# bwfbowen/muax

Hardware: AMD Instinct MI355X
Metric: batched act() env-steps/sec at num_simulations=50 (higher is better)
Workload: dtype f32; 1 GPU; cartpole: 4096 roots/GPU, obs 4, MLP embed 8, A=2, support 10, num_simulations=50, dirichlet 0.25/0.3, tiebreak=threefry, temperature 1; roots_per_gpu=4096, num_simulations=50, parallelism=roots sharded x1, no collective, backend=none (one rank), launcher=none

## Files before the change

muax_amd/_jit.py:

```python
from __future__ import annotations

import ctypes as C
import hashlib
import os
import subprocess

from . import _build

JIT_DIR = os.path.join(_build.LIB_DIR, "jit")
_SOURCES = ["mz_fused_jit.hip", "mz_fused_group.inc", "mz_fused_launch.h", "mz_fused.cuh", "mz_spec.cuh", "mz_host.h"]
_loaded = {}
_failed = set()
_TRAIN_SOURCES = ["mz_train_jit.hip", "mz_train_launch.h", "mz_train.cuh", "mz_spec.cuh", "mz_host.h"]
PLAN_VERSION = 2
last_build_log = None


def _ceil_log2(n: int) -> int:
    return 0 if n <= 1 else 1 + _ceil_log2((n + 1) // 2)


def lds_bytes(A: int, E: int, NMAX: int, WAVES: int, long_paths: bool = False, gumbel: bool = True) -> int:
    selw = ((2 * A + 3) // 4) * 4
    st0 = selw + (4 if (gumbel or not long_paths) else 3)
    path0 = st0 + (5 if gumbel else 4) * A + (E if (E <= 16 and not long_paths) else 0)
    entry = 8 if _ceil_log2(NMAX) + max(1, _ceil_log2(A)) <= 8 else 16
    pathw = (NMAX * entry + 31) // 32
    ns = (path0 + (0 if long_paths else pathw)) | 1
    tree = ((ns * NMAX + 3) // 4) * 4 + (((A + 3) // 4) * 4 if (long_paths and gumbel) else 0)
# ... 214 lines not shown
```

muax_amd/csrc/mz_act.hip:

```cpp
#include <hip/hip_runtime.h>

#include <cstdlib>
#include <cstring>

#define MZ_NO_STEP_KERNELS
#include "mz_handle.h"
#include "mz_fused_launch.h"
#include "mz_wide_launch.h"

using mzh::fail;

template <class Call>
static int dispatch_with_scratch(mzs_handle* h, mz::FusedParams& p, int* rc, Call call) {
  const size_t BN = (size_t)h->cfg.batch * (h->cfg.num_simulations + 1);
  *rc = call();
  for (int tries = 0; tries < 2 && (*rc == mz::kNeedEmbScratch || *rc >= mz::kNeedPathScratch); ++tries) {
    if (*rc == mz::kNeedEmbScratch) {
      MZS_HIP(h, hipMalloc(reinterpret_cast<void**>(&h->fused_emb), BN * h->cfg.embed_dim * sizeof(float)));
      p.emb_scratch = h->fused_emb;
    } else {
      const int words = *rc - mz::kNeedPathScratch;
      if (h->fused_path) MZS_HIP(h, hipFree(h->fused_path));
      h->fused_path = nullptr;
      h->fused_path_words = 0;
// ... 16 lines not shown
  if (!h->have_weights) return fail(h, MZS_E_INVALID, "mzs_act_mlp: call mzs_mlp_set_weights first");
  if (!a->obs || !a->action || !a->action_weights || !a->root_value)
    return fail(h, MZS_E_INVALID, "mzs_act_mlp: obs/action/action_weights/root_value must be set");
  const mzs_config& c = h->cfg;
  if (c.policy == 0 && !a->dirichlet_noise && a->dirichlet_fraction != 0.0f)
    return fail(h, MZS_E_INVALID, "mzs_act_mlp: dirichlet_fraction != 0 needs dirichlet_noise");
  if (c.num_simulations > mz::kMaxSims) {
    if (h->allow_generic) return mzh::act_mlp_generic(h, a, stream_);
    return fail(h, MZS_E_UNSUPPORTED, "mzs_act_mlp: no fused kernel instance for num_simulations > 256; use the generic route "
                                      "(mzs_mlp_allow_generic) or the step-wise path");
  }
  hipStream_t stream = static_cast<hipStream_t>(stream_);
  MZS_HIP(h, hipSetDevice(c.device));

  mz::FusedParams p;
  memset(&p, 0, sizeof p);
  p.obs = a->obs; p.dirichlet_noise = a->dirichlet_noise; p.invalid = a->invalid_actions; p.gumbel = a->gumbel;
  const mzs_mlp_weights& w = h->w;
  mzh::copy_weights(w, p);
  p.action = a->action; p.action_weights = a->action_weights; p.root_value = a->root_value;
  p.search_value = a->search_value; p.depth_sum = a->depth_sum;
  if (a->tree) {
    const mzs_tree_view& t = *a->tree;
    const void* const* tp = reinterpret_cast<const void* const*>(&t);
    for (int i = 0; i < 12; ++i)
      if (!tp[i]) return fail(h, MZS_E_INVALID, "mzs_act_mlp: tree view has a null array");
    p.t_node_visits = t.node_visits; p.t_raw_values = t.raw_values; p.t_node_values = t.node_values;
    p.t_parents = t.parents; p.t_action_from_parent = t.action_from_parent;
    p.t_children_index = t.children_index; p.t_children_prior_logits = t.children_prior_logits;
    p.t_children_values = t.children_values; p.t_children_visits = t.children_visits;
    p.t_children_rewards = t.children_rewards; p.t_children_discounts = t.children_discounts;
// ... 6 lines not shown
  p.dirichlet_fraction = a->dirichlet_fraction; p.discount = w.discount; p.temperature = a->temperature;
  p.global_batch = (uint64_t)c.global_batch; p.root_offset = (uint64_t)c.root_offset;
  p.prof = h->prof;
  p.emb_scratch = p.export_tree ? nullptr : h->fused_emb;
  if (c.policy == 1) {
    if (!h->fused_table) {
      const std::vector<int32_t> table = mzh::visit_table(c.max_num_considered_actions, c.num_simulations);
      MZS_HIP(h, hipMalloc(reinterpret_cast<void**>(&h->fused_table), table.size() * sizeof(int32_t)));
      MZS_HIP(h, hipMemcpy(h->fused_table, table.data(), table.size() * sizeof(int32_t), hipMemcpyHostToDevice));
    }
    p.visit_table = h->fused_table;
    p.max_considered = c.max_num_considered_actions;
    p.gumbel_scale = c.gumbel_scale;
    mzh::h_split(a->key, 2, 1, p.k_gumbel);
  }
  mzh::derive_keys(a->key, h->cfg.num_simulations, h->k_sample, h->sim_keys.data());
  p.k_sample[0] = h->k_sample[0]; p.k_sample[1] = h->k_sample[1];
  memcpy(p.sim_keys, h->sim_keys.data(), sizeof(uint32_t) * 2 * (size_t)c.num_simulations);

  const int A = c.num_actions, E = c.embed_dim, F = 2 * w.support_size + 1, N = c.num_simulations + 1;
  p.F = F;
  const int mode = c.policy == 1 ? (c.qtransform == 1 ? 3 : 2) : (c.tiebreak ? 1 : 0);
  std::vector<mz::FusedDispatch> groups = {mz::fused_dispatch_g0, mz::fused_dispatch_g1, mz::fused_dispatch_g2,
                                           mz::fused_dispatch_g3, mz::fused_dispatch_g4};
  mz::jit_dispatchers(mode, &groups);
  if (h->allow_generic && getenv("MZS_FORCE_GENERIC") != nullptr) return mzh::act_mlp_generic(h, a, stream_);
  for (int compact = (c.batch > 16 * h->cu_count) ? 1 : 0; compact >= 0; --compact) {
    p.path_scratch = h->fused_path;
    p.path_words = h->fused_path_words;
    for (size_t gi = 0; gi < groups.size(); ++gi) {
      std::string err;
      int rc = 0;
      auto call = [&] { return groups[gi](mode, c.device, p, stream, A, E, F, N, compact != 0, &err); };
      if (int e = dispatch_with_scratch(h, p, &rc, call)) return e;
      if (rc == mz::kNoFusedInstance) continue;
      if (rc != MZS_OK) return fail(h, rc, "mzs_act_mlp: %s", err.c_str());
      return MZS_OK;
    }
  }
  if (mode >= 2 ? h->allow_wide_gumbel : h->allow_wide) {
    std::string err;
    int rc = 0;
    auto call = [&] { return mz::wide_dispatch(mode, h->allow_wide_gumbel, c.device, p, stream, A, E, F, &err); };
    if (int e = dispatch_with_scratch(h, p, &rc, call)) return e;
    if (rc == MZS_OK) return MZS_OK;
    if (rc != mz::kNoFusedInstance) return fail(h, rc, "mzs_act_mlp: %s", err.c_str());
  }
  if (h->allow_generic) return mzh::act_mlp_generic(h, a, stream_);
// ... 75 lines not shown
```

muax_amd/csrc/mz_api.hip:

```cpp
#include <hip/hip_runtime.h>

#include <cstdio>
#include <cstring>
#include <mutex>

#define MZ_NO_STEP_KERNELS
#include "mz_handle.h"
#include "mz_fused_launch.h"

namespace {

thread_local std::string g_create_error;

std::mutex g_jit_mutex;
std::vector<mz::FusedDispatch> g_jit_dispatch;
std::vector<mz::FusedDispatch> g_jit_dispatch_muzero;
struct JitTrain { int A, E, F; mzh::JitTrainLaunch launch; };
std::vector<JitTrain> g_jit_train;

}

int mzh::fail(mzs_handle* h, int code, const char* fmt, const char* a) {
  char buf[512];
  snprintf(buf, sizeof buf, fmt, a);
// ... 75 lines not shown
  return MZS_OK;
}
int mzs_mlp_allow_wide_gumbel(mzs_handle* h, int32_t allow) {
  if (!h) return MZS_E_INVALID;
  h->allow_wide_gumbel = allow != 0;
  return MZS_OK;
}

int mzs_destroy(mzs_handle* h) {
  if (!h) return MZS_OK;
  hipSetDevice(h->cfg.device);
  h->step.release();
  if (h->fused_table) hipFree(h->fused_table);
  if (h->fused_emb) hipFree(h->fused_emb);
  if (h->fused_path) hipFree(h->fused_path);
  if (h->jump_slab) hipFree(h->jump_slab);
  if (h->host_in) hipHostFree(h->host_in);
  if (h->host_out) hipHostFree(h->host_out);
  if (h->dev_noise) hipFree(h->dev_noise);
  if (h->gen_scratch) hipFree(h->gen_scratch);
  delete h;
  return MZS_OK;
}

int mzs_mlp_set_weights(mzs_handle* h, const mzs_mlp_weights* w) {
  if (!h) return MZS_E_INVALID;
  if (!w || w->struct_size != (int32_t)sizeof(mzs_mlp_weights))
    return fail(h, MZS_E_INVALID, "mzs_mlp_set_weights: null or size mismatch (ABI)");
  const float* const* ptrs = &w->repr_w;
  for (int i = 0; i < 18; ++i)
    if (!ptrs[i]) return fail(h, MZS_E_INVALID, "mzs_mlp_set_weights: null weight pointer");
  if (w->obs_dim <= 0 || w->support_size <= 0) return fail(h, MZS_E_INVALID, "mzs_mlp_set_weights: obs_dim/support_size");
  h->w = *w;
  h->have_weights = true;
  return MZS_OK;
}

static int register_dispatch(std::vector<mz::FusedDispatch>& list, void* dispatch, int32_t jit_abi) {
  if (!dispatch) return fail(nullptr, MZS_E_INVALID, "mzs_register_fused_dispatch: null");
  if (jit_abi != mzs_fused_jit_abi()) return fail(nullptr, MZS_E_INVALID, "mzs_register_fused_dispatch: the side library was built from other sources (ABI)");
  std::lock_guard<std::mutex> lock(g_jit_mutex);
  for (auto f : list)
    if (reinterpret_cast<void*>(f) == dispatch) return MZS_OK;
  list.push_back(reinterpret_cast<mz::FusedDispatch>(dispatch));
  return MZS_OK;
}
int mzs_register_fused_dispatch(void* dispatch, int32_t jit_abi) { return register_dispatch(g_jit_dispatch, dispatch, jit_abi); }
int mzs_register_fused_dispatch_muzero(void* dispatch, int32_t jit_abi) {
  return register_dispatch(g_jit_dispatch_muzero, dispatch, jit_abi);
// ... 4 lines not shown
```

muax_amd/csrc/mz_fused.cuh:

```cuda
#pragma once
#include "mz_spec.cuh"

#pragma clang fp contract(off)

namespace mz {

#ifdef MZ_PROFILE
#define MZ_TICK(slot)                                  \
  do {                                                 \
    uint64_t now_ = __builtin_amdgcn_s_memtime();      \
    prof_acc[slot] += now_ - prof_t;                   \
    prof_t = now_;                                     \
  } while (0)
#define MZ_TICKW(slot)                                 \
  do {                                                 \
    asm volatile("s_waitcnt vmcnt(0) lgkmcnt(0)" ::: "memory"); \
    MZ_TICK(slot);                                     \
  } while (0)
#else
#define MZ_TICK(slot) do {} while (0)
#define MZ_TICKW(slot) do {} while (0)
#endif

constexpr int kMaxSims = 256;
constexpr int kHidden = 16;

struct FusedParams {
  const float* obs;
  const float* dirichlet_noise;
  const uint8_t* invalid;
  const float* gumbel;
  const float *repr_w, *repr_b;
  const float *pv_w1, *pv_b1, *pv_w2, *pv_b2;
  const float *pp_w1, *pp_b1, *pp_w2, *pp_b2;
  const float *dr_w1, *dr_b1, *dr_w2, *dr_b2;
  const float *dn_w1, *dn_b1, *dn_w2, *dn_b2;
  int32_t* action;
  float* action_weights;
  float* root_value;
  float* search_value;
  int32_t* depth_sum;
  int32_t* t_node_visits; float* t_raw_values; float* t_node_values;
  int32_t* t_parents; int32_t* t_action_from_parent;
  int32_t* t_children_index; float* t_children_prior_logits; float* t_children_values;
  int32_t* t_children_visits; float* t_children_rewards; float* t_children_discounts;
  float* t_embeddings;
  float* emb_scratch;
  int32_t* path_scratch;
  int32_t B, obs_dim, S, max_depth, support, F, pred_on_parent, export_tree;
  float pb_c_init, pb_c_base, dirichlet_fraction, discount, temperature;
  uint64_t global_batch, root_offset;
  uint32_t k_sample[2];
  const int32_t* visit_table;
  int32_t max_considered;
  float gumbel_scale;
  uint32_t k_gumbel[2];
  uint32_t sim_keys[kMaxSims][2];
  uint64_t* prof;
  int32_t path_words;
};

template <int A_, int E_, int FS_, int NMAX_, int MODE_, int WAVES_ = 4, int REC_ = 0>
struct FusedCfg {
  static_assert(REC_ >= 0 && REC_ <= 2, "record kind");
  static constexpr bool PH_ = REC_ != 0;
  static constexpr bool PH = PH_;
  static constexpr bool LONG = REC_ == 2;
  static constexpr int WAVES = WAVES_, THREADS = 64 * WAVES_;
  static constexpr int A = A_, E = E_, FS = FS_, NMAX = NMAX_, MODE = MODE_;
  static_assert(FS_ == 2 || FS_ == 4, "support logits are handled as one or two packed pairs of lane slots");
  static constexpr bool TB = MODE_ == 1;
  static constexpr bool GUMBEL = MODE_ >= 2;
  static constexpr int QT = MODE_ == 3 ? 1 : 0;
  static constexpr int H = kHidden;
  static constexpr int ES = (E + 15) / 16;
  static constexpr bool L1_DPP = E_ > 16 && E_ % 8 == 0;
  static constexpr bool L2_BLOCK = L1_DPP && FS_ == 2 && (E_ + 15) / 16 == 2 && A_ <= 16;
  static constexpr bool PK = PH_ && E_ > 16 && !LONG;
  static_assert(!PK || (A_ <= 4 && NMAX_ <= 128 && MODE_ < 2), "packed record: four byte-sized children, MuZero policy");
  static constexpr int SEL0 = 0, SELW = PK ? 1 + A : ((2 * A + 3) / 4) * 4;
  static constexpr int HDR0 = SELW, JUMP = HDR0 + 2;
  static constexpr bool RAW_OK = !(PH_ && MODE_ != 3);
  static constexpr int HDRW = RAW_OK ? 4 : 3;
  static constexpr int ST0 = HDR0 + HDRW, STW = MODE_ >= 2 ? 5 : 4, ST_LOGIT = 4;
  static constexpr bool EMB_LDS = E_ <= 16 && !LONG;
  static constexpr int EMB0 = PK ? ST0 + 3 * A + 1 : ST0 + STW * A;
  static constexpr int off_score(int a) { return PK ? SEL0 + 1 + a : SEL0 + 2 * a + 1; }
  static constexpr int off_prob(int a) { return PK ? ST0 + a : ST0 + STW * a; }
  static constexpr int off_val(int a) { return PK ? ST0 + A + a : ST0 + STW * a + 1; }
  static constexpr int off_rew(int a) { return PK ? ST0 + 2 * A + a : ST0 + STW * a + 3; }
  static constexpr int off_logit(int a) { return ST0 + STW * a + ST_LOGIT; }
  static constexpr int VIS0 = ST0 + 3 * A;
  static MZ_DEV void load_cidx(const int* ndi, int (&cidx)[A]) {
// ... 60 lines not shown

template <int NIN, int NOUT>
struct RowLinear {
  static constexpr int IS = (NIN + 15) / 16, OS = (NOUT + 15) / 16;
  float w[NIN][OS];
  float b[OS];
  MZ_DEV void load(const float* __restrict__ W, const float* __restrict__ Bv, int j) {
#pragma unroll
    for (int t = 0; t < OS; ++t) {
      int k = j + 16 * t;
      b[t] = k < NOUT ? Bv[k] : 0.0f;
#pragma unroll
      for (int i = 0; i < NIN; ++i) w[i][t] = k < NOUT ? W[i * NOUT + k] : 0.0f;
    }
  }
  MZ_DEV void apply(const float (&x)[IS], float (&y)[OS]) const {
#pragma unroll
    for (int t = 0; t < OS; ++t) y[t] = 0.0f;
    StaticFor<0, NIN>::run([&](auto ic) {
      constexpr int i = decltype(ic)::value;
      float xb = bcast<(i & 15)>(x[i >> 4]);
#pragma unroll
      for (int t = 0; t < OS; ++t) y[t] = __builtin_fmaf(xb, w[i][t], y[t]);
    });
#pragma unroll
    for (int t = 0; t < OS; ++t) y[t] = y[t] + b[t];
  }
};

template <int NIN, int OS>
struct RowLinearRT {
  float w[NIN][OS];
  float b[OS];
  MZ_DEV void load(const float* __restrict__ W, const float* __restrict__ Bv, int j, int nout) {
#pragma unroll
    for (int t = 0; t < OS; ++t) {
      int k = j + 16 * t;
      b[t] = k < nout ? Bv[k] : 0.0f;
#pragma unroll
      for (int i = 0; i < NIN; ++i) w[i][t] = k < nout ? W[i * nout + k] : 0.0f;
    }
  }
};

template <int E, int A>
struct RowLinearOneHot2 {
  f32x2 w[E];
  f32x2 wa[A];
  f32x2 b;
  MZ_DEV void load(const float* __restrict__ W0, const float* __restrict__ B0, const float* __restrict__ W1,
                   const float* __restrict__ B1, int j) {
    b = (f32x2){B0[j], B1[j]};
    StaticFor<0, E>::run([&](auto ic) {
      constexpr int i = decltype(ic)::value;
      w[i] = (f32x2){W0[i * kHidden + j], W1[i * kHidden + j]};
    });
    StaticFor<0, A>::run([&](auto ac) {
      constexpr int a = decltype(ac)::value;
      wa[a] = (f32x2){W0[(E + a) * kHidden + j], W1[(E + a) * kHidden + j]};
    });
  }
};

template <int E>
struct RowLinearPair {
  f32x2 w[E];
  f32x2 b;
  MZ_DEV void load(const float* __restrict__ W0, const float* __restrict__ B0, const float* __restrict__ W1,
                   const float* __restrict__ B1, int j) {
    b = (f32x2){B0[j], B1[j]};
    StaticFor<0, E>::run([&](auto ic) {
      constexpr int i = decltype(ic)::value;
      w[i] = (f32x2){W0[i * kHidden + j], W1[i * kHidden + j]};
    });
  }
};

template <int N>
MZ_DEV void row_softmax(const float (&x)[(N + 15) / 16], int j, float (&p)[(N + 15) / 16]) {
  constexpr int NSLOT = (N + 15) / 16;
  constexpr int STEPS = N >= 16 ? 4 : ceil_log2(N);
  float m = -INFINITY;
#pragma unroll
  for (int t = 0; t < NSLOT; ++t) m = (j + 16 * t < N) ? fmaxf(m, x[t]) : m;
  m = row_max<STEPS>(m);
  float e[NSLOT];
  float part = 0.0f;
#pragma unroll
// ... 59 lines not shown
      s[0] = q.x;
      s[1] = q.y;
      return;
    }
  }
#pragma unroll
  for (int t = 0; t < NSLOT; ++t) s[t] = (s[t] - mn) / scale;
}

struct RowBias2 {
  f32x2 b;
  MZ_DEV void load(const float* __restrict__, const float* __restrict__ B0, const float* __restrict__,
                   const float* __restrict__ B1, int j) {
    b = (f32x2){B0[j], B1[j]};
  }
};

template <bool COND, class T, class F> struct PickType { using type = T; };
template <class T, class F> struct PickType<false, T, F> { using type = F; };

template <class C>
struct Nets {
  typename PickType<C::PK, RowBias2, RowLinearPair<C::E>>::type p1;
  RowLinearRT<kHidden, C::FS> pv2;
  RowLinear<kHidden, C::A> pp2;
  typename PickType<C::PK, RowBias2, RowLinearOneHot2<C::E, C::A>>::type d1;
  RowLinearRT<kHidden, C::FS> dr2;
  RowLinear<kHidden, C::E> dn2;
  const float* wlds = nullptr;

// ... 3 lines not shown
      for (int idx = tid; idx < (E / 2) * 16; idx += C::THREADS) {
        const int i = 2 * (idx >> 4), jj = idx & 15;
        *reinterpret_cast<float4*>(wl + 4 * idx) = make_float4(p.pv_w1[i * kHidden + jj], p.pp_w1[i * kHidden + jj],
                                                               p.pv_w1[(i + 1) * kHidden + jj], p.pp_w1[(i + 1) * kHidden + jj]);
      }
      float* wd = wl + C::W1P_WORDS;
      for (int idx = tid; idx < ((RD + 1) / 2) * 16; idx += C::THREADS) {
        const int i = 2 * (idx >> 4), jj = idx & 15;
        const bool two = i + 1 < RD;
        *reinterpret_cast<float4*>(wd + 4 * idx) = make_float4(p.dr_w1[i * kHidden + jj], p.dn_w1[i * kHidden + jj],
                                                               two ? p.dr_w1[(i + 1) * kHidden + jj] : 0.0f,
                                                               two ? p.dn_w1[(i + 1) * kHidden + jj] : 0.0f);
      }
    }
  }
  template <int WHICH>
  MZ_DEV f32x2 first_layers_lds(const float (&x)[C::ES]) const {
    static_assert(C::E % 8 == 0, "eight inputs per statement");
    const float* base = wlds + (WHICH ? C::W1P_WORDS : 0);
    float h0 = 0.0f, h1 = 0.0f;
    StaticFor<0, C::E / 8>::run([&](auto ic) {
      constexpr int i = 8 * decltype(ic)::value;
      f32x2 w[8];
#pragma unroll
      for (int q = 0; q < 4; ++q) {
        const float4 v = *reinterpret_cast<const float4*>(base + (i / 2 + q) * 64);
        w[2 * q] = (f32x2){v.x, v.y};
        w[2 * q + 1] = (f32x2){v.z, v.w};
      }
      fmac_bcast_pair8<(i & 15), (i & 15) == 0>(h0, h1, x[i >> 4], w);
// ... 2 lines not shown
  }
  MZ_DEV f32x2 first_p(const float (&x)[C::ES]) const {
    if constexpr (C::PK) return first_layers_lds<0>(x);
    else return first_layers(x, p1.w);
  }
  MZ_DEV f32x2 first_d(const float (&x)[C::ES]) const {
    if constexpr (C::PK) return first_layers_lds<1>(x);
    else return first_layers(x, d1.w);
  }

  MZ_DEV void load(const FusedParams& p, int j) {
    p1.load(p.pv_w1, p.pv_b1, p.pp_w1, p.pp_b1, j);
    pv2.load(p.pv_w2, p.pv_b2, j, p.F); pp2.load(p.pp_w2, p.pp_b2, j);
    d1.load(p.dr_w1, p.dr_b1, p.dn_w1, p.dn_b1, j);
    dr2.load(p.dr_w2, p.dr_b2, j, p.F); dn2.load(p.dn_w2, p.dn_b2, j);
  }
  template <class W>
  MZ_DEV f32x2 first_layers(const float (&x)[C::ES], const W& w) const {
    if constexpr (C::L1_DPP) {
      static_assert(C::E % 8 == 0, "eight inputs per statement");
      float h0 = 0.0f, h1 = 0.0f;
      StaticFor<0, C::E / 8>::run([&](auto ic) {
        constexpr int i = 8 * decltype(ic)::value;
        fmac_bcast_pair8<(i & 15), (i & 15) == 0>(h0, h1, x[i >> 4], &w[i]);
      });
      return (f32x2){h0, h1};
    } else {
      f32x2 h = splat2(0.0f);
      StaticFor<0, C::E>::run([&](auto ic) {
        constexpr int i = decltype(ic)::value;
// ... 323 lines not shown
    x[a] = logit[a] + qv[a];
    mxl = fmaxf(mxl, logit[a]);
  }
  softmax_inlane<A>(x, pr);
#pragma unroll
  for (int a = 0; a < A; ++a) {
    float r = fmaxf((gum[a] + (logit[a] - mxl)) + qv[a], -1e9f);
    r = r + (vis[a] == considered_visit ? 0.0f : -INFINITY);
    r = ((inv_bits >> a) & 1u) ? -INFINITY : r;
    const float in = pr[a] - (float)vis[a] / (float)(1 + sum_visits);
    sc[a] = is_root ? r : in;
  }
}

template <class C>
__global__ __launch_bounds__(C::THREADS, (C::PH && !C::LONG) ? 2 : 1) void mz_act_fused_kernel(const FusedParams p) {
  constexpr int A = C::A, E = C::E, NS = C::NS;
  extern __shared__ __attribute__((aligned(16))) float lds[];
  if constexpr (!C::PK) asm volatile("; keep AGPRs allocatable" ::: "a0");
  const int tid = threadIdx.x;
  const int lane = tid & 63;
  const int j = lane & 15;
  const int root_in_wg = (tid >> 6) * 4 + (lane >> 4);
  const int r_raw = blockIdx.x * C::ROOTS_PER_WG + root_in_wg;
  const int r = r_raw < p.B ? r_raw : p.B - 1;

#ifdef MZ_PROFILE
  uint64_t prof_acc[16] = {0, 0, 0, 0, 0, 0, 0, 0, 0, 0, 0, 0, 0, 0, 0, 0};
  uint64_t prof_t = __builtin_amdgcn_s_memtime();
#endif
  Nets<C> nets;
  if constexpr (C::PK) {
    nets.load(p, j);
    nets.wlds = lds + C::TBL_WORDS + 4 * j;
  }
  float* tbl = lds;
  for (int i = tid; i < C::TBL_WORDS / 2; i += C::THREADS) {
    tbl[2 * i] = puct_scale(i, p.pb_c_init, p.pb_c_base);
    tbl[2 * i + 1] = i > 0 ? 1.0f / (float)i : 0.0f;
  }
  Nets<C>::fill_lds(p, lds + C::TBL_WORDS, tid);
  __syncthreads();

  float* tree = lds + C::TBL_WORDS + C::WLDS_WORDS + root_in_wg * C::ROOT_WORDS;
  int* itree = reinterpret_cast<int*>(tree);
  const uint64_t rg = p.root_offset + (uint64_t)r;
  const int S = p.S;
  const int max_depth = p.max_depth > 0 ? p.max_depth : S;
  const int N = S + 1;
  const int support = p.support;
  const bool ex = p.export_tree != 0;

  float* gemb = C::EMB_LDS ? nullptr : (ex ? p.t_embeddings : p.emb_scratch) + (size_t)r * N * E;

  int32_t* gpath = C::PH ? p.path_scratch + (size_t)r * N * C::PATHW : nullptr;

  if constexpr (!C::PK) nets.load(p, j);
  {
    int4* q4 = reinterpret_cast<int4*>(itree);
    const int nq = (N * NS + 3) / 4;
    for (int q = j; q < nq; q += 16) q4[q] = make_int4(0, 0, 0, 0);
    for (int n = j; n < N; n += 16) {
      if constexpr (C::PK) itree[n * NS + C::SEL0] = -1;
      else {
#pragma unroll
        for (int a = 0; a < A; ++a) itree[n * NS + C::SEL0 + 2 * a] = -1;
      }
    }
  }
  if (ex) {
    for (int n = j; n < N; n += 16) {
      size_t o = (size_t)r * N + n;
      p.t_raw_values[o] = 0.0f;
      p.t_parents[o] = -1;
      p.t_action_from_parent[o] = -1;
    }
    for (int i = j; i < N * A; i += 16) p.t_children_prior_logits[(size_t)r * N * A + i] = 0.0f;
    if constexpr (!C::EMB_LDS)
      for (int i = j; i < N * E; i += 16) gemb[i] = 0.0f;
  }

  float s[C::ES];
  {
    const float* ob = p.obs + (size_t)r * p.obs_dim;
#pragma unroll
    for (int t = 0; t < C::ES; ++t) {
      int k = j + 16 * t;
      float acc = 0.0f;
      {
        const int kc = k < E ? k : 0;
        int i = 0;
        for (; i + 4 <= p.obs_dim; i += 4) {
          float o4[4], w4[4];
#pragma unroll
          for (int q = 0; q < 4; ++q) {
            o4[q] = ob[i + q];
            w4[q] = p.repr_w[(i + q) * E + kc];
          }
#pragma unroll
          for (int q = 0; q < 4; ++q) acc = __builtin_fmaf(o4[q], w4[q], acc);
        }
        for (; i < p.obs_dim; ++i) acc = __builtin_fmaf(ob[i], p.repr_w[i * E + kc], acc);
        acc = acc + p.repr_b[kc];
      }
      s[t] = k < E ? acc : 0.0f;
    }
    row_min_max_normalize<E>(s, j);
  }
  float v0, pl0;
  nets.predict(s, j, support, p.F, v0, pl0);
  uint32_t inv_bits = 0;
  if (p.invalid != nullptr) {
#pragma unroll
    for (int a = 0; a < A; ++a) inv_bits |= p.invalid[(size_t)r * A + a] ? (1u << a) : 0u;
  }
  int ncons = 0;
  int root_jw;
  {
    float lg, pq[1];
    if constexpr (!C::GUMBEL) {
      float x[1] = {pl0}, pr[1];
      row_softmax<A>(x, j, pr);
      float nz = (p.dirichlet_noise != nullptr && j < A) ? p.dirichlet_noise[(size_t)r * A + j] : 0.0f;
      float keep = 1.0f - p.dirichlet_fraction;
      float noisy = keep * pr[0] + p.dirichlet_fraction * nz;
      lg = log_pos(fmaxf(noisy, kFltTiny));
      if (p.invalid != nullptr) {
        float mx = row_max<4>(j < A ? lg : -INFINITY);
        lg = ((inv_bits >> j) & 1u) ? kFltLowest : lg - mx;
      }
      float lx[1] = {lg};
      row_softmax<A>(lx, j, pq);
    } else {
      lg = pl0;
      if (inv_bits != 0) {
        float mx = row_max<4>(j < A ? lg : -INFINITY);
        lg = ((inv_bits >> j) & 1u) ? kFltLowest : lg - mx;
      }
// ... 546 lines not shown
```

muax_amd/csrc/mz_fused_group.inc:

```
#include <mutex>

#ifndef MZ_INSTANCES_FILE
#define MZ_INSTANCES_FILE "mz_instances.def"
#endif
#include "../../include/mzsearch.h"
#include "mz_fused_launch.h"
#include "mz_host.h"

namespace mz {
namespace {

template <class C>
int launch_fused(int device, const FusedParams& p, hipStream_t stream, std::string* err) {
  static mzh::LdsGrant granted;
  if (!granted.covers(device, (size_t)C::LDS_BYTES)) {
    const hipError_t attr_err = hipFuncSetAttribute(reinterpret_cast<const void*>(&mz_act_fused_kernel<C>),
                                                    hipFuncAttributeMaxDynamicSharedMemorySize, C::LDS_BYTES);
    if (attr_err != hipSuccess) {
      *err = std::string("hipFuncSetAttribute: ") + hipGetErrorString(attr_err);
      return MZS_E_RUNTIME;
    }
    granted.note(device, (size_t)C::LDS_BYTES);
  }
  const int grid = (p.B + C::ROOTS_PER_WG - 1) / C::ROOTS_PER_WG;
  hipLaunchKernelGGL(mz_act_fused_kernel<C>, dim3(grid), dim3(C::THREADS), C::LDS_BYTES, stream, p);
  const hipError_t e = hipGetLastError();
  if (e != hipSuccess) {
    *err = std::string("fused kernel launch: ") + hipGetErrorString(e);
    return MZS_E_RUNTIME;
  }
  return MZS_OK;
}

#ifndef MZ_FUSED_MUZERO_ONLY
#define MZ_FUSED_MUZERO_ONLY 0
#endif

template <int A, int E, int FS, int NMAX, int WAVES, int PH>
int dispatch_mode(int mode, int device, const FusedParams& p, hipStream_t stream, std::string* err) {
  using C0 = FusedCfg<A, E, FS, NMAX, 0, WAVES, PH>;
  constexpr bool kMuZeroOnly = (PH && !C0::LONG) || MZ_FUSED_MUZERO_ONLY;
  if (kMuZeroOnly && mode >= 2) return kNoFusedInstance;
  if constexpr (PH) {
    if (p.path_scratch == nullptr || p.path_words < C0::PATHW) return kNeedPathScratch + C0::PATHW;
  }
  if constexpr (!C0::EMB_LDS) {
    if (!p.export_tree && p.emb_scratch == nullptr) return kNeedEmbScratch;
  }
  if constexpr (kMuZeroOnly) {
    if (mode == 1) return launch_fused<FusedCfg<A, E, FS, NMAX, 1, WAVES, PH>>(device, p, stream, err);
    return launch_fused<FusedCfg<A, E, FS, NMAX, 0, WAVES, PH>>(device, p, stream, err);
  } else {
    switch (mode) {
      case 3: return launch_fused<FusedCfg<A, E, FS, NMAX, 3, WAVES, PH>>(device, p, stream, err);
      case 2: return launch_fused<FusedCfg<A, E, FS, NMAX, 2, WAVES, PH>>(device, p, stream, err);
      case 1: return launch_fused<FusedCfg<A, E, FS, NMAX, 1, WAVES, PH>>(device, p, stream, err);
      default: return launch_fused<FusedCfg<A, E, FS, NMAX, 0, WAVES, PH>>(device, p, stream, err);
    }
  }
}

template <int G>
int dispatch_group(int mode, int device, const FusedParams& p, hipStream_t stream, int A, int E, int F, int N,
                   bool compact, std::string* err) {
#define MZS_INST(G_, A_, E_, FS_, NMAX_, WAVES_, PH_)                                                   \
  if constexpr (G_ == G)                                                                                \
    if (A == A_ && E == E_ && F > 16 * (FS_ - 2) && F > 16 && F <= 16 * FS_ && N <= NMAX_ &&                      \
        ((int)(PH_) == 2 ? !compact : compact == ((int)(PH_) == 1)))                                              \
      return dispatch_mode<A_, E_, FS_, NMAX_, WAVES_, PH_>(mode, device, p, stream, err);
#include MZ_INSTANCES_FILE
#undef MZS_INST
  return kNoFusedInstance;
}

}

#define MZ_CAT_(a, b) a##b
#define MZ_CAT(a, b) MZ_CAT_(a, b)
int MZ_CAT(fused_dispatch_g, MZ_FUSED_GROUP)(int mode, int device, const FusedParams& p, hipStream_t stream, int A, int E,
                                             int F, int N, bool compact, std::string* err) {
  return dispatch_group<MZ_FUSED_GROUP>(mode, device, p, stream, A, E, F, N, compact, err);
}

}
```

muax_amd/csrc/mz_fused_launch.h:

```cpp
#pragma once
#include <string>
#include <vector>

#include "mz_fused.cuh"

namespace mz {
constexpr int kNoFusedInstance = 1;
constexpr int kNeedPathScratch = 1000;
constexpr int kNeedEmbScratch = 2;
using FusedDispatch = int (*)(int mode, int device, const FusedParams& p, hipStream_t stream, int A, int E, int F,
                              int N, bool compact, std::string* err);
int fused_dispatch_g0(int mode, int device, const FusedParams& p, hipStream_t stream, int A, int E, int F, int N, bool compact, std::string* err);
int fused_dispatch_g1(int mode, int device, const FusedParams& p, hipStream_t stream, int A, int E, int F, int N, bool compact, std::string* err);
int fused_dispatch_g2(int mode, int device, const FusedParams& p, hipStream_t stream, int A, int E, int F, int N, bool compact, std::string* err);
int fused_dispatch_g3(int mode, int device, const FusedParams& p, hipStream_t stream, int A, int E, int F, int N, bool compact, std::string* err);
int fused_dispatch_g4(int mode, int device, const FusedParams& p, hipStream_t stream, int A, int E, int F, int N, bool compact, std::string* err);
void jit_dispatchers(int mode, std::vector<FusedDispatch>* out);
}
```

muax_amd/csrc/mz_handle.h:

```cpp
#pragma once
#include <string>
#include <vector>

#include "mz_host.h"
#include "mz_keys.h"
#include "mz_step_jump.cuh"

struct mzs_handle {
  mzs_config cfg;
  std::string err;
  bool have_weights = false;
  mzs_mlp_weights w;
  mz::StepState step;
  uint32_t k_sample[2] = {0, 0};
  std::vector<uint32_t> sim_keys;
  uint64_t* prof = nullptr;
  int32_t* fused_table = nullptr;
  float* fused_emb = nullptr;
  int32_t* fused_path = nullptr;
  int fused_path_words = 0;
  int cu_count = 0;
  void* host_in = nullptr; void* host_out = nullptr; void* dev_noise = nullptr;
  size_t host_in_bytes = 0;
  mz::JumpArgs jump = {nullptr, nullptr, nullptr, nullptr};
  void* jump_slab = nullptr;
  bool use_jump = false;
  int jump_roots = 0;
  bool allow_generic = false;
  float* gen_scratch = nullptr;
  bool allow_wide = false;
  bool allow_wide_gumbel = false;
};

namespace mzh {

// ... 13 lines not shown
```

muax_amd/csrc/mz_host.h:

```cpp
#pragma once
#include <hip/hip_runtime.h>

#include <atomic>
#include <cstdio>
#include <string>

#include "../../include/mzsearch.h"

#define MZS_HIP(h, call)                                                                            \
  do {                                                                                              \
    hipError_t e_ = (call);                                                                         \
    if (e_ != hipSuccess) return mzh::fail(h, MZS_E_RUNTIME, #call ": %s", hipGetErrorString(e_));  \
  } while (0)

namespace mz {
struct StepArgs;
struct JumpArgs;
}
namespace mzh {
int step_view(mzs_handle* h, mz::StepArgs* sa, mz::JumpArgs* ja, int* policy, const char* who, int* device = nullptr);
int fail(mzs_handle* h, int code, const char* fmt, const char* a = "");
using JitTrainLaunch = int (*)(const void* train_params, void* stream, char* err, int errlen);
JitTrainLaunch jit_train_instance(int A, int E, int F);
struct LdsGrant {
  std::atomic<size_t> have[64];
  bool covers(int device, size_t lds) const {
    return device >= 0 && device < 64 && have[device].load(std::memory_order_acquire) >= lds;
  }
  void note(int device, size_t lds) {
    if (device < 0 || device >= 64) return;
    size_t cur = have[device].load(std::memory_order_relaxed);
    while (cur < lds && !have[device].compare_exchange_weak(cur, lds, std::memory_order_release)) {
    }
  }
};
inline int check_device(int device, const char* who) {
  int ndev = 0;
  if (hipGetDeviceCount(&ndev) != hipSuccess || ndev <= 0)
    return fail(nullptr, MZS_E_NODEVICE, "%s: no HIP device (this library has no CPU fallback)", who);
  if (device < 0 || device >= ndev) return fail(nullptr, MZS_E_INVALID, "%s: bad device ordinal", who);
  return MZS_OK;
}
inline int select_device(int device, const char* who) {
  if (int rc = check_device(device, who)) return rc;
  MZS_HIP(nullptr, hipSetDevice(device));
  return MZS_OK;
}
}
```

Measured before the change: 34.77 million env-steps/s.

## Cache a prepacked weight and PUCT-table image across act calls

```diff
diff --git a/muax_amd/_jit.py b/muax_amd/_jit.py
--- a/muax_amd/_jit.py
+++ b/muax_amd/_jit.py
@@ -12,7 +12,7 @@
 _loaded = {}
 _failed = set()
 _TRAIN_SOURCES = ["mz_train_jit.hip", "mz_train_launch.h", "mz_train.cuh", "mz_spec.cuh", "mz_host.h"]
-PLAN_VERSION = 2
+PLAN_VERSION = 3
 last_build_log = None
 
 
diff --git a/muax_amd/csrc/mz_act.hip b/muax_amd/csrc/mz_act.hip
--- a/muax_amd/csrc/mz_act.hip
+++ b/muax_amd/csrc/mz_act.hip
@@ -1,5 +1,6 @@
 #include <hip/hip_runtime.h>
 
+#include <cstddef>
 #include <cstdlib>
 #include <cstring>
 
@@ -54,7 +55,7 @@
   MZS_HIP(h, hipSetDevice(c.device));
 
   mz::FusedParams p;
-  memset(&p, 0, sizeof p);
+  memset(&p, 0, offsetof(mz::FusedParams, sim_keys));
   p.obs = a->obs; p.dirichlet_noise = a->dirichlet_noise; p.invalid = a->invalid_actions; p.gumbel = a->gumbel;
   const mzs_mlp_weights& w = h->w;
   mzh::copy_weights(w, p);
@@ -91,9 +92,7 @@
     p.gumbel_scale = c.gumbel_scale;
     mzh::h_split(a->key, 2, 1, p.k_gumbel);
   }
-  mzh::derive_keys(a->key, h->cfg.num_simulations, h->k_sample, h->sim_keys.data());
-  p.k_sample[0] = h->k_sample[0]; p.k_sample[1] = h->k_sample[1];
-  memcpy(p.sim_keys, h->sim_keys.data(), sizeof(uint32_t) * 2 * (size_t)c.num_simulations);
+  mzh::derive_keys(a->key, c.num_simulations, p.k_sample, &p.sim_keys[0][0]);
 
   const int A = c.num_actions, E = c.embed_dim, F = 2 * w.support_size + 1, N = c.num_simulations + 1;
   p.F = F;
@@ -108,7 +107,7 @@
     for (size_t gi = 0; gi < groups.size(); ++gi) {
       std::string err;
       int rc = 0;
-      auto call = [&] { return groups[gi](mode, c.device, p, stream, A, E, F, N, compact != 0, &err); };
+      auto call = [&] { return groups[gi](mode, c.device, p, &h->fused_image, stream, A, E, F, N, compact != 0, &err); };
       if (int e = dispatch_with_scratch(h, p, &rc, call)) return e;
       if (rc == mz::kNoFusedInstance) continue;
       if (rc != MZS_OK) return fail(h, rc, "mzs_act_mlp: %s", err.c_str());
diff --git a/muax_amd/csrc/mz_api.hip b/muax_amd/csrc/mz_api.hip
--- a/muax_amd/csrc/mz_api.hip
+++ b/muax_amd/csrc/mz_api.hip
@@ -113,6 +113,7 @@
   if (h->fused_table) hipFree(h->fused_table);
   if (h->fused_emb) hipFree(h->fused_emb);
   if (h->fused_path) hipFree(h->fused_path);
+  if (h->fused_image.dev) hipFree(h->fused_image.dev);
   if (h->jump_slab) hipFree(h->jump_slab);
   if (h->host_in) hipHostFree(h->host_in);
   if (h->host_out) hipHostFree(h->host_out);
@@ -132,6 +133,7 @@
   if (w->obs_dim <= 0 || w->support_size <= 0) return fail(h, MZS_E_INVALID, "mzs_mlp_set_weights: obs_dim/support_size");
   h->w = *w;
   h->have_weights = true;
+  h->fused_image.valid = false;
   return MZS_OK;
 }
 
diff --git a/muax_amd/csrc/mz_fused.cuh b/muax_amd/csrc/mz_fused.cuh
--- a/muax_amd/csrc/mz_fused.cuh
+++ b/muax_amd/csrc/mz_fused.cuh
@@ -22,42 +22,53 @@
 #define MZ_TICKW(slot) do {} while (0)
 #endif
 
+#ifndef MZ_WEIGHTS_FIRST_PLAIN
+#define MZ_WEIGHTS_FIRST_PLAIN 0
+#endif
+#ifndef MZ_INPUTS_FIRST_PLAIN
+#define MZ_INPUTS_FIRST_PLAIN 0
+#endif
+#ifndef MZ_INPUTS_FIRST_PACKED
+#define MZ_INPUTS_FIRST_PACKED 0
+#endif
+
 constexpr int kMaxSims = 256;
 constexpr int kHidden = 16;
 
 struct FusedParams {
+  const float* image;
   const float* obs;
   const float* dirichlet_noise;
   const uint8_t* invalid;
   const float* gumbel;
+  int32_t* action;
+  float* action_weights;
+  float* root_value;
+  float* search_value;
+  int32_t* depth_sum;
+  int32_t B, obs_dim, S, max_depth, support, F, pred_on_parent, export_tree;
+  float pb_c_init, pb_c_base, dirichlet_fraction, discount, temperature;
+  int32_t path_words;
+  uint64_t global_batch, root_offset;
+  uint32_t k_sample[2];
+  float* emb_scratch;
+  int32_t* path_scratch;
+  const int32_t* visit_table;
+  int32_t max_considered;
+  float gumbel_scale;
+  uint32_t k_gumbel[2];
+  uint64_t* prof;
+  int32_t* t_node_visits; float* t_raw_values; float* t_node_values;
+  int32_t* t_parents; int32_t* t_action_from_parent;
+  int32_t* t_children_index; float* t_children_prior_logits; float* t_children_values;
+  int32_t* t_children_visits; float* t_children_rewards; float* t_children_discounts;
+  float* t_embeddings;
   const float *repr_w, *repr_b;
   const float *pv_w1, *pv_b1, *pv_w2, *pv_b2;
   const float *pp_w1, *pp_b1, *pp_w2, *pp_b2;
   const float *dr_w1, *dr_b1, *dr_w2, *dr_b2;
   const float *dn_w1, *dn_b1, *dn_w2, *dn_b2;
-  int32_t* action;
-  float* action_weights;
-  float* root_value;
-  float* search_value;
-  int32_t* depth_sum;
-  int32_t* t_node_visits; float* t_raw_values; float* t_node_values;
-  int32_t* t_parents; int32_t* t_action_from_parent;
-  int32_t* t_children_index; float* t_children_prior_logits; float* t_children_values;
-  int32_t* t_children_visits; float* t_children_rewards; float* t_children_discounts;
-  float* t_embeddings;
-  float* emb_scratch;
-  int32_t* path_scratch;
-  int32_t B, obs_dim, S, max_depth, support, F, pred_on_parent, export_tree;
-  float pb_c_init, pb_c_base, dirichlet_fraction, discount, temperature;
-  uint64_t global_batch, root_offset;
-  uint32_t k_sample[2];
-  const int32_t* visit_table;
-  int32_t max_considered;
-  float gumbel_scale;
-  uint32_t k_gumbel[2];
   uint32_t sim_keys[kMaxSims][2];
-  uint64_t* prof;
-  int32_t path_words;
 };
 
 template <int A_, int E_, int FS_, int NMAX_, int MODE_, int WAVES_ = 4, int REC_ = 0>
@@ -77,6 +88,8 @@
   static constexpr bool L1_DPP = E_ > 16 && E_ % 8 == 0;
   static constexpr bool L2_BLOCK = L1_DPP && FS_ == 2 && (E_ + 15) / 16 == 2 && A_ <= 16;
   static constexpr bool PK = PH_ && E_ > 16 && !LONG;
+  static constexpr bool WEIGHTS_FIRST = MZ_WEIGHTS_FIRST_PLAIN ? true : PK;
+  static constexpr bool INPUTS_FIRST = PK ? MZ_INPUTS_FIRST_PACKED : MZ_INPUTS_FIRST_PLAIN;
   static_assert(!PK || (A_ <= 4 && NMAX_ <= 128 && MODE_ < 2), "packed record: four byte-sized children, MuZero policy");
   static constexpr int SEL0 = 0, SELW = PK ? 1 + A : ((2 * A + 3) / 4) * 4;
   static constexpr int HDR0 = SELW, JUMP = HDR0 + 2;
@@ -167,6 +180,17 @@
       for (int i = 0; i < NIN; ++i) w[i][t] = k < NOUT ? W[i * NOUT + k] : 0.0f;
     }
   }
+  static constexpr int WORDS = (NIN + 1) * OS;
+  template <class V>
+  MZ_DEV void each(V& v) {
+#pragma unroll
+    for (int t = 0; t < OS; ++t) b[t] = v(b[t]);
+#pragma unroll
+    for (int i = 0; i < NIN; ++i) {
+#pragma unroll
+      for (int t = 0; t < OS; ++t) w[i][t] = v(w[i][t]);
+    }
+  }
   MZ_DEV void apply(const float (&x)[IS], float (&y)[OS]) const {
 #pragma unroll
     for (int t = 0; t < OS; ++t) y[t] = 0.0f;
@@ -192,6 +216,17 @@
       b[t] = k < nout ? Bv[k] : 0.0f;
 #pragma unroll
       for (int i = 0; i < NIN; ++i) w[i][t] = k < nout ? W[i * nout + k] : 0.0f;
+    }
+  }
+  static constexpr int WORDS = (NIN + 1) * OS;
+  template <class V>
+  MZ_DEV void each(V& v) {
+#pragma unroll
+    for (int t = 0; t < OS; ++t) b[t] = v(b[t]);
+#pragma unroll
+    for (int i = 0; i < NIN; ++i) {
+#pragma unroll
+      for (int t = 0; t < OS; ++t) w[i][t] = v(w[i][t]);
     }
   }
 };
@@ -213,6 +248,22 @@
       wa[a] = (f32x2){W0[(E + a) * kHidden + j], W1[(E + a) * kHidden + j]};
     });
   }
+  static constexpr int WORDS = 2 * (E + A + 1);
+  template <class V>
+  MZ_DEV void each(V& v) {
+    b.x = v(b.x);
+    b.y = v(b.y);
+    StaticFor<0, E>::run([&](auto ic) {
+      constexpr int i = decltype(ic)::value;
+      w[i].x = v(w[i].x);
+      w[i].y = v(w[i].y);
+    });
+    StaticFor<0, A>::run([&](auto ac) {
+      constexpr int a = decltype(ac)::value;
+      wa[a].x = v(wa[a].x);
+      wa[a].y = v(wa[a].y);
+    });
+  }
 };
 
 template <int E>
@@ -225,6 +276,17 @@
     StaticFor<0, E>::run([&](auto ic) {
       constexpr int i = decltype(ic)::value;
       w[i] = (f32x2){W0[i * kHidden + j], W1[i * kHidden + j]};
+    });
+  }
+  static constexpr int WORDS = 2 * (E + 1);
+  template <class V>
+  MZ_DEV void each(V& v) {
+    b.x = v(b.x);
+    b.y = v(b.y);
+    StaticFor<0, E>::run([&](auto ic) {
+      constexpr int i = decltype(ic)::value;
+      w[i].x = v(w[i].x);
+      w[i].y = v(w[i].y);
     });
   }
 };
@@ -314,6 +376,33 @@
                    const float* __restrict__ B1, int j) {
     b = (f32x2){B0[j], B1[j]};
   }
+  static constexpr int WORDS = 2;
+  template <class V>
+  MZ_DEV void each(V& v) {
+    b.x = v(b.x);
+    b.y = v(b.y);
+  }
+};
+
+struct ImagePut {
+  float* base;
+  int k = 0;
+  MZ_DEV float operator()(float x) {
+    base[(k >> 2) * 64 + (k & 3)] = x;
+    ++k;
+    return x;
+  }
+};
+struct ImageTake {
+  const float* base;
+  float4 cur = make_float4(0.0f, 0.0f, 0.0f, 0.0f);
+  int k = 0;
+  MZ_DEV float operator()(float) {
+    if ((k & 3) == 0) cur = *reinterpret_cast<const float4*>(base + (k >> 2) * 64);
+    const float x = (k & 3) == 0 ? cur.x : (k & 3) == 1 ? cur.y : (k & 3) == 2 ? cur.z : cur.w;
+    ++k;
+    return x;
+  }
 };
 
 template <bool COND, class T, class F> struct PickType { using type = T; };
@@ -347,6 +436,12 @@
       }
     }
   }
+  static MZ_DEV void copy_lds(const float* __restrict__ src, float* wl, int tid) {
+    if constexpr (C::PK) {
+      for (int idx = tid; idx < C::WLDS_WORDS / 4; idx += C::THREADS)
+        reinterpret_cast<float4*>(wl)[idx] = reinterpret_cast<const float4*>(src)[idx];
+    }
+  }
   template <int WHICH>
   MZ_DEV f32x2 first_layers_lds(const float (&x)[C::ES]) const {
     static_assert(C::E % 8 == 0, "eight inputs per statement");
@@ -379,6 +474,19 @@
     pv2.load(p.pv_w2, p.pv_b2, j, p.F); pp2.load(p.pp_w2, p.pp_b2, j);
     d1.load(p.dr_w1, p.dr_b1, p.dn_w1, p.dn_b1, j);
     dr2.load(p.dr_w2, p.dr_b2, j, p.F); dn2.load(p.dn_w2, p.dn_b2, j);
+  }
+  using P1 = typename PickType<C::PK, RowBias2, RowLinearPair<C::E>>::type;
+  using D1 = typename PickType<C::PK, RowBias2, RowLinearOneHot2<C::E, C::A>>::type;
+  static constexpr int WORDS = P1::WORDS + 2 * RowLinearRT<kHidden, C::FS>::WORDS + RowLinear<kHidden, C::A>::WORDS +
+                               D1::WORDS + RowLinear<kHidden, C::E>::WORDS;
+  static constexpr int CHUNKS = (WORDS + 3) / 4;
+  template <class V>
+  MZ_DEV void each(V& v) {
+    p1.each(v); pv2.each(v); pp2.each(v); d1.each(v); dr2.each(v); dn2.each(v);
+  }
+  MZ_DEV void load_image(const float* __restrict__ wimg, int j) {
+    ImageTake take{wimg + 4 * j};
+    each(take);
   }
   template <class W>
   MZ_DEV f32x2 first_layers(const float (&x)[C::ES], const W& w) const {
@@ -732,7 +840,49 @@
 }
 
 template <class C>
+struct FusedImage {
+  static constexpr int TBL0 = 0;
+  static constexpr int W0 = C::TBL_WORDS;
+  static constexpr int WL0 = W0 + Nets<C>::CHUNKS * 64;
+  static constexpr int REPR0 = WL0 + C::WLDS_WORDS;
+  static constexpr int REPR_ROWS = 16 * C::ES;
+  static_assert(W0 % 4 == 0 && WL0 % 4 == 0 && REPR0 % 4 == 0, "16-byte blocks");
+  static __host__ __device__ constexpr int repr_row_words(int obs_dim) { return 4 + ((obs_dim + 3) & ~3); }
+  static __host__ __device__ constexpr size_t words(int obs_dim) {
+    return (size_t)REPR0 + (size_t)REPR_ROWS * (size_t)repr_row_words(obs_dim);
+  }
+};
+
+template <class C>
+__global__ __launch_bounds__(C::THREADS) void mz_fused_image_kernel(const FusedParams p, float* __restrict__ img) {
+  using I = FusedImage<C>;
+  const int tid = threadIdx.x;
+  for (int i = tid; i < C::TBL_WORDS / 2; i += C::THREADS) {
+    img[I::TBL0 + 2 * i] = puct_scale(i, p.pb_c_init, p.pb_c_base);
+    img[I::TBL0 + 2 * i + 1] = i > 0 ? 1.0f / (float)i : 0.0f;
+  }
+  if (tid < 16) {
+    Nets<C> nets;
+    nets.load(p, tid);
+    ImagePut put{img + I::W0 + 4 * tid};
+    nets.each(put);
+  }
+  Nets<C>::fill_lds(p, img + I::WL0, tid);
+  const int rw = I::repr_row_words(p.obs_dim);
+  for (int idx = tid; idx < I::REPR_ROWS * rw; idx += C::THREADS) {
+    const int k = idx / rw, c = idx - k * rw;
+    float v = 0.0f;
+    if (k < C::E) {
+      if (c == 0) v = p.repr_b[k];
+      else if (c >= 4 && c - 4 < p.obs_dim) v = p.repr_w[(c - 4) * C::E + k];
+    }
+    img[I::REPR0 + idx] = v;
+  }
+}
+
+template <class C>
 __global__ __launch_bounds__(C::THREADS, (C::PH && !C::LONG) ? 2 : 1) void mz_act_fused_kernel(const FusedParams p) {
+  using I = FusedImage<C>;
   constexpr int A = C::A, E = C::E, NS = C::NS;
   extern __shared__ __attribute__((aligned(16))) float lds[];
   if constexpr (!C::PK) asm volatile("; keep AGPRs allocatable" ::: "a0");
@@ -747,17 +897,16 @@
   uint64_t prof_acc[16] = {0, 0, 0, 0, 0, 0, 0, 0, 0, 0, 0, 0, 0, 0, 0, 0};
   uint64_t prof_t = __builtin_amdgcn_s_memtime();
 #endif
+  const float* __restrict__ img = p.image;
   Nets<C> nets;
-  if constexpr (C::PK) {
-    nets.load(p, j);
-    nets.wlds = lds + C::TBL_WORDS + 4 * j;
+  if constexpr (C::WEIGHTS_FIRST) {
+    nets.load_image(img + I::W0, j);
+    if constexpr (C::PK) nets.wlds = lds + C::TBL_WORDS + 4 * j;
   }
   float* tbl = lds;
-  for (int i = tid; i < C::TBL_WORDS / 2; i += C::THREADS) {
-    tbl[2 * i] = puct_scale(i, p.pb_c_init, p.pb_c_base);
-    tbl[2 * i + 1] = i > 0 ? 1.0f / (float)i : 0.0f;
-  }
-  Nets<C>::fill_lds(p, lds + C::TBL_WORDS, tid);
+  for (int i = tid; i < C::TBL_WORDS / 4; i += C::THREADS)
+    reinterpret_cast<float4*>(tbl)[i] = reinterpret_cast<const float4*>(img + I::TBL0)[i];
+  Nets<C>::copy_lds(img + I::WL0, lds + C::TBL_WORDS, tid);
   __syncthreads();
 
   float* tree = lds + C::TBL_WORDS + C::WLDS_WORDS + root_in_wg * C::ROOT_WORDS;
@@ -773,7 +922,7 @@
 
   int32_t* gpath = C::PH ? p.path_scratch + (size_t)r * N * C::PATHW : nullptr;
 
-  if constexpr (!C::PK) nets.load(p, j);
+  if constexpr (!C::WEIGHTS_FIRST) nets.load_image(img + I::W0, j);
   {
     int4* q4 = reinterpret_cast<int4*>(itree);
     const int nq = (N * NS + 3) / 4;
@@ -798,6 +947,15 @@
       for (int i = j; i < N * E; i += 16) gemb[i] = 0.0f;
   }
 
+  uint32_t inv_bits = 0;
+  float nz = 0.0f;
+  if constexpr (C::INPUTS_FIRST) {
+    if (p.invalid != nullptr) {
+#pragma unroll
+      for (int a = 0; a < A; ++a) inv_bits |= p.invalid[(size_t)r * A + a] ? (1u << a) : 0u;
+    }
+    if constexpr (!C::GUMBEL) nz = (p.dirichlet_noise != nullptr && j < A) ? p.dirichlet_noise[(size_t)r * A + j] : 0.0f;
+  }
   float s[C::ES];
   {
     const float* ob = p.obs + (size_t)r * p.obs_dim;
@@ -806,20 +964,21 @@
       int k = j + 16 * t;
       float acc = 0.0f;
       {
-        const int kc = k < E ? k : 0;
+        const float* __restrict__ col = img + I::REPR0 + (size_t)k * I::repr_row_words(p.obs_dim);
+        const float bias = col[0];
         int i = 0;
         for (; i + 4 <= p.obs_dim; i += 4) {
-          float o4[4], w4[4];
-#pragma unroll
-          for (int q = 0; q < 4; ++q) {
-            o4[q] = ob[i + q];
-            w4[q] = p.repr_w[(i + q) * E + kc];
-          }
-#pragma unroll
-          for (int q = 0; q < 4; ++q) acc = __builtin_fmaf(o4[q], w4[q], acc);
+          float o4[4];
+#pragma unroll
+          for (int q = 0; q < 4; ++q) o4[q] = ob[i + q];
+          const float4 w4 = *reinterpret_cast<const float4*>(col + 4 + i);
+          acc = __builtin_fmaf(o4[0], w4.x, acc);
+          acc = __builtin_fmaf(o4[1], w4.y, acc);
+          acc = __builtin_fmaf(o4[2], w4.z, acc);
+          acc = __builtin_fmaf(o4[3], w4.w, acc);
         }
-        for (; i < p.obs_dim; ++i) acc = __builtin_fmaf(ob[i], p.repr_w[i * E + kc], acc);
-        acc = acc + p.repr_b[kc];
+        for (; i < p.obs_dim; ++i) acc = __builtin_fmaf(ob[i], col[4 + i], acc);
+        acc = acc + bias;
       }
       s[t] = k < E ? acc : 0.0f;
     }
@@ -827,10 +986,11 @@
   }
   float v0, pl0;
   nets.predict(s, j, support, p.F, v0, pl0);
-  uint32_t inv_bits = 0;
-  if (p.invalid != nullptr) {
-#pragma unroll
-    for (int a = 0; a < A; ++a) inv_bits |= p.invalid[(size_t)r * A + a] ? (1u << a) : 0u;
+  if constexpr (!C::INPUTS_FIRST) {
+    if (p.invalid != nullptr) {
+#pragma unroll
+      for (int a = 0; a < A; ++a) inv_bits |= p.invalid[(size_t)r * A + a] ? (1u << a) : 0u;
+    }
   }
   int ncons = 0;
   int root_jw;
@@ -839,7 +999,7 @@
     if constexpr (!C::GUMBEL) {
       float x[1] = {pl0}, pr[1];
       row_softmax<A>(x, j, pr);
-      float nz = (p.dirichlet_noise != nullptr && j < A) ? p.dirichlet_noise[(size_t)r * A + j] : 0.0f;
+      if constexpr (!C::INPUTS_FIRST) nz = (p.dirichlet_noise != nullptr && j < A) ? p.dirichlet_noise[(size_t)r * A + j] : 0.0f;
       float keep = 1.0f - p.dirichlet_fraction;
       float noisy = keep * pr[0] + p.dirichlet_fraction * nz;
       lg = log_pos(fmaxf(noisy, kFltTiny));
diff --git a/muax_amd/csrc/mz_fused_group.inc b/muax_amd/csrc/mz_fused_group.inc
--- a/muax_amd/csrc/mz_fused_group.inc
+++ b/muax_amd/csrc/mz_fused_group.inc
@@ -11,7 +11,43 @@
 namespace {
 
 template <class C>
-int launch_fused(int device, const FusedParams& p, hipStream_t stream, std::string* err) {
+int ensure_image(FusedParams& p, mzh::FusedImageSlot* slot, hipStream_t stream, std::string* err) {
+  static const char instance = 0;
+  if (!slot->serves(&instance, p.F, p.obs_dim, p.pb_c_init, p.pb_c_base)) {
+    const size_t words = FusedImage<C>::words(p.obs_dim);
+    slot->valid = false;
+    if (slot->cap_words < words) {
+      if (slot->dev) hipFree(slot->dev);
+      slot->dev = nullptr;
+      slot->cap_words = 0;
+      const hipError_t me = hipMalloc(reinterpret_cast<void**>(&slot->dev), words * sizeof(float));
+      if (me != hipSuccess) {
+        (void)hipGetLastError();
+        slot->dev = nullptr;
+        *err = std::string("launch image: hipMalloc: ") + hipGetErrorString(me);
+        return MZS_E_RUNTIME;
+      }
+      slot->cap_words = words;
+    }
+    hipError_t e = hipMemsetAsync(slot->dev, 0, words * sizeof(float), stream);
+    if (e == hipSuccess) {
+      float* img = slot->dev;
+      void* args[] = {&p, &img};
+      e = hipLaunchKernel(reinterpret_cast<const void*>(&mz_fused_image_kernel<C>), dim3(1), dim3(C::THREADS), args, 0, stream);
+    }
+    if (e != hipSuccess) {
+      (void)hipGetLastError();
+      *err = std::string("launch image build: ") + hipGetErrorString(e);
+      return MZS_E_RUNTIME;
+    }
+    slot->built(&instance, p.F, p.obs_dim, p.pb_c_init, p.pb_c_base);
+  }
+  p.image = slot->dev;
+  return MZS_OK;
+}
+
+template <class C>
+int launch_fused(int device, FusedParams& p, mzh::FusedImageSlot* slot, hipStream_t stream, std::string* err) {
   static mzh::LdsGrant granted;
   if (!granted.covers(device, (size_t)C::LDS_BYTES)) {
     const hipError_t attr_err = hipFuncSetAttribute(reinterpret_cast<const void*>(&mz_act_fused_kernel<C>),
@@ -22,10 +58,13 @@
     }
     granted.note(device, (size_t)C::LDS_BYTES);
   }
+  if (int rc = ensure_image<C>(p, slot, stream, err)) return rc;
   const int grid = (p.B + C::ROOTS_PER_WG - 1) / C::ROOTS_PER_WG;
-  hipLaunchKernelGGL(mz_act_fused_kernel<C>, dim3(grid), dim3(C::THREADS), C::LDS_BYTES, stream, p);
-  const hipError_t e = hipGetLastError();
+  void* args[] = {&p};
+  const hipError_t e = hipLaunchKernel(reinterpret_cast<const void*>(&mz_act_fused_kernel<C>), dim3(grid), dim3(C::THREADS),
+                                       args, C::LDS_BYTES, stream);
   if (e != hipSuccess) {
+    (void)hipGetLastError();
     *err = std::string("fused kernel launch: ") + hipGetErrorString(e);
     return MZS_E_RUNTIME;
   }
@@ -37,7 +76,7 @@
 #endif
 
 template <int A, int E, int FS, int NMAX, int WAVES, int PH>
-int dispatch_mode(int mode, int device, const FusedParams& p, hipStream_t stream, std::string* err) {
+int dispatch_mode(int mode, int device, FusedParams& p, mzh::FusedImageSlot* slot, hipStream_t stream, std::string* err) {
   using C0 = FusedCfg<A, E, FS, NMAX, 0, WAVES, PH>;
   constexpr bool kMuZeroOnly = (PH && !C0::LONG) || MZ_FUSED_MUZERO_ONLY;
   if (kMuZeroOnly && mode >= 2) return kNoFusedInstance;
@@ -48,26 +87,26 @@
     if (!p.export_tree && p.emb_scratch == nullptr) return kNeedEmbScratch;
   }
   if constexpr (kMuZeroOnly) {
-    if (mode == 1) return launch_fused<FusedCfg<A, E, FS, NMAX, 1, WAVES, PH>>(device, p, stream, err);
-    return launch_fused<FusedCfg<A, E, FS, NMAX, 0, WAVES, PH>>(device, p, stream, err);
+    if (mode == 1) return launch_fused<FusedCfg<A, E, FS, NMAX, 1, WAVES, PH>>(device, p, slot, stream, err);
+    return launch_fused<FusedCfg<A, E, FS, NMAX, 0, WAVES, PH>>(device, p, slot, stream, err);
   } else {
     switch (mode) {
-      case 3: return launch_fused<FusedCfg<A, E, FS, NMAX, 3, WAVES, PH>>(device, p, stream, err);
-      case 2: return launch_fused<FusedCfg<A, E, FS, NMAX, 2, WAVES, PH>>(device, p, stream, err);
-      case 1: return launch_fused<FusedCfg<A, E, FS, NMAX, 1, WAVES, PH>>(device, p, stream, err);
-      default: return launch_fused<FusedCfg<A, E, FS, NMAX, 0, WAVES, PH>>(device, p, stream, err);
+      case 3: return launch_fused<FusedCfg<A, E, FS, NMAX, 3, WAVES, PH>>(device, p, slot, stream, err);
+      case 2: return launch_fused<FusedCfg<A, E, FS, NMAX, 2, WAVES, PH>>(device, p, slot, stream, err);
+      case 1: return launch_fused<FusedCfg<A, E, FS, NMAX, 1, WAVES, PH>>(device, p, slot, stream, err);
+      default: return launch_fused<FusedCfg<A, E, FS, NMAX, 0, WAVES, PH>>(device, p, slot, stream, err);
     }
   }
 }
 
 template <int G>
-int dispatch_group(int mode, int device, const FusedParams& p, hipStream_t stream, int A, int E, int F, int N,
+int dispatch_group(int mode, int device, FusedParams& p, mzh::FusedImageSlot* slot, hipStream_t stream, int A, int E, int F, int N,
                    bool compact, std::string* err) {
 #define MZS_INST(G_, A_, E_, FS_, NMAX_, WAVES_, PH_)                                                   \
   if constexpr (G_ == G)                                                                                \
     if (A == A_ && E == E_ && F > 16 * (FS_ - 2) && F > 16 && F <= 16 * FS_ && N <= NMAX_ &&                      \
         ((int)(PH_) == 2 ? !compact : compact == ((int)(PH_) == 1)))                                              \
-      return dispatch_mode<A_, E_, FS_, NMAX_, WAVES_, PH_>(mode, device, p, stream, err);
+      return dispatch_mode<A_, E_, FS_, NMAX_, WAVES_, PH_>(mode, device, p, slot, stream, err);
 #include MZ_INSTANCES_FILE
 #undef MZS_INST
   return kNoFusedInstance;
@@ -77,9 +116,9 @@
 
 #define MZ_CAT_(a, b) a##b
 #define MZ_CAT(a, b) MZ_CAT_(a, b)
-int MZ_CAT(fused_dispatch_g, MZ_FUSED_GROUP)(int mode, int device, const FusedParams& p, hipStream_t stream, int A, int E,
+int MZ_CAT(fused_dispatch_g, MZ_FUSED_GROUP)(int mode, int device, FusedParams& p, mzh::FusedImageSlot* slot, hipStream_t stream, int A, int E,
                                              int F, int N, bool compact, std::string* err) {
-  return dispatch_group<MZ_FUSED_GROUP>(mode, device, p, stream, A, E, F, N, compact, err);
+  return dispatch_group<MZ_FUSED_GROUP>(mode, device, p, slot, stream, A, E, F, N, compact, err);
 }
 
 }
diff --git a/muax_amd/csrc/mz_fused_launch.h b/muax_amd/csrc/mz_fused_launch.h
--- a/muax_amd/csrc/mz_fused_launch.h
+++ b/muax_amd/csrc/mz_fused_launch.h
@@ -3,17 +3,18 @@
 #include <vector>
 
 #include "mz_fused.cuh"
+#include "mz_host.h"
 
 namespace mz {
 constexpr int kNoFusedInstance = 1;
 constexpr int kNeedPathScratch = 1000;
 constexpr int kNeedEmbScratch = 2;
-using FusedDispatch = int (*)(int mode, int device, const FusedParams& p, hipStream_t stream, int A, int E, int F,
+using FusedDispatch = int (*)(int mode, int device, FusedParams& p, mzh::FusedImageSlot* image, hipStream_t stream, int A, int E, int F,
                               int N, bool compact, std::string* err);
-int fused_dispatch_g0(int mode, int device, const FusedParams& p, hipStream_t stream, int A, int E, int F, int N, bool compact, std::string* err);
-int fused_dispatch_g1(int mode, int device, const FusedParams& p, hipStream_t stream, int A, int E, int F, int N, bool compact, std::string* err);
-int fused_dispatch_g2(int mode, int device, const FusedParams& p, hipStream_t stream, int A, int E, int F, int N, bool compact, std::string* err);
-int fused_dispatch_g3(int mode, int device, const FusedParams& p, hipStream_t stream, int A, int E, int F, int N, bool compact, std::string* err);
-int fused_dispatch_g4(int mode, int device, const FusedParams& p, hipStream_t stream, int A, int E, int F, int N, bool compact, std::string* err);
+int fused_dispatch_g0(int mode, int device, FusedParams& p, mzh::FusedImageSlot* image, hipStream_t stream, int A, int E, int F, int N, bool compact, std::string* err);
+int fused_dispatch_g1(int mode, int device, FusedParams& p, mzh::FusedImageSlot* image, hipStream_t stream, int A, int E, int F, int N, bool compact, std::string* err);
+int fused_dispatch_g2(int mode, int device, FusedParams& p, mzh::FusedImageSlot* image, hipStream_t stream, int A, int E, int F, int N, bool compact, std::string* err);
+int fused_dispatch_g3(int mode, int device, FusedParams& p, mzh::FusedImageSlot* image, hipStream_t stream, int A, int E, int F, int N, bool compact, std::string* err);
+int fused_dispatch_g4(int mode, int device, FusedParams& p, mzh::FusedImageSlot* image, hipStream_t stream, int A, int E, int F, int N, bool compact, std::string* err);
 void jit_dispatchers(int mode, std::vector<FusedDispatch>* out);
 }
diff --git a/muax_amd/csrc/mz_handle.h b/muax_amd/csrc/mz_handle.h
--- a/muax_amd/csrc/mz_handle.h
+++ b/muax_amd/csrc/mz_handle.h
@@ -19,6 +19,7 @@
   float* fused_emb = nullptr;
   int32_t* fused_path = nullptr;
   int fused_path_words = 0;
+  mzh::FusedImageSlot fused_image;
   int cu_count = 0;
   void* host_in = nullptr; void* host_out = nullptr; void* dev_noise = nullptr;
   size_t host_in_bytes = 0;
diff --git a/muax_amd/csrc/mz_host.h b/muax_amd/csrc/mz_host.h
--- a/muax_amd/csrc/mz_host.h
+++ b/muax_amd/csrc/mz_host.h
@@ -34,6 +34,28 @@
     }
   }
 };
+struct FusedImageSlot {
+  float* dev = nullptr;
+  size_t cap_words = 0;
+  bool valid = false;
+  const void* instance = nullptr;
+  int32_t F = 0, obs_dim = 0;
+  uint32_t pb_c_init = 0, pb_c_base = 0;
+  static uint32_t bits(float f) {
+    uint32_t u;
+    static_assert(sizeof u == sizeof f, "");
+    __builtin_memcpy(&u, &f, sizeof u);
+    return u;
+  }
+  bool serves(const void* inst, int32_t F_, int32_t obs_dim_, float c_init, float c_base) const {
+    return valid && dev != nullptr && instance == inst && F == F_ && obs_dim == obs_dim_ && pb_c_init == bits(c_init) &&
+           pb_c_base == bits(c_base);
+  }
+  void built(const void* inst, int32_t F_, int32_t obs_dim_, float c_init, float c_base) {
+    instance = inst; F = F_; obs_dim = obs_dim_; pb_c_init = bits(c_init); pb_c_base = bits(c_base);
+    valid = true;
+  }
+};
 inline int check_device(int device, const char* who) {
   int ndev = 0;
   if (hipGetDeviceCount(&ndev) != hipSuccess || ndev <= 0)
```

After: 35.08 million env-steps/s (median of 6 runs). No clear change (+0.9%).
